# simplerr/rust-renderer

Hardware: AMD Instinct MI355X
Metric: Mrays/s (path rays: primary + bounce + sun-shadow + light-shadow) at 1920x1080, 20 spp = 20 frames x 1 spp; camera and sun at rest, the one-off builds of the camera grid and the sun grid outside the timed region (value_with_grid_builds charges them to these frames, value_tree_walk uses neither grid) (higher is better)
Workload: dtype f32

## Files before the change

rust-renderer_amd/csrc/context.hip:

```cpp
#include <hip/hip_runtime.h>
#include <rccl/rccl.h>
#include <dlfcn.h>

#include <algorithm>
#include <atomic>
#include <cstdlib>
#include <cmath>
#include <cstdio>
#include <cstring>
#include <string>
#include <vector>

#include "bvh.h"
#include "context_internal.h"
#include "context_state.h"
#include "device_scan.h"
#include "device_types.h"
#include "texture_layout.h"
#include "utopian_hip.h"

using namespace uh;

namespace {
std::string g_create_error;
// ... 344 lines not shown
   HIP_TRY(c, s.create(need));
   return UH_OK;
}

static int enqueue_path_trace(uh_ctx* c, Slot& s, const FrameParams& frame) {
   FrameParams fp = frame;
   LaunchCfg lc = cfg(c);
   lc.stream = s.stream;
   if (fp.batch_frames == 1) {
      lc.closest_blocks_per_cu = std::min(lc.closest_blocks_per_cu, uh_ctx::kSingleFrameBlocksPerCu);
      lc.shadow_blocks_per_cu = std::min(lc.shadow_blocks_per_cu, uh_ctx::kSingleFrameBlocksPerCu);
   }
   Control* ctl = s.control.p;
   DeviceStats* st = c->dstats.p;
   for (uint32_t smp = 0; smp < fp.samples_per_frame; smp++) {
      HIP_TRY(c, hipMemsetAsync(ctl, 0, sizeof(Control), s.stream));
      uint32_t slot = 0;
      launch_generate(lc, fp, s.ps, ctl, smp);
      const bool gpu_idle = !c->last_acc || hipEventQuery(c->last_acc) == hipSuccess;
      const bool fused = c->fused_bounces && fp.batch_frames == 1 && fp.num_bounces >= 2 && fp.num_bounces <= 64 && s.ps.shard_cap < (1u << 23) &&
                         ((gpu_idle && fp.n_owned <= uh_ctx::kFusedMaxPaths) || c->fused_always);
      const bool fused_sun0 = fused && fp.sun_shadow_enabled == 1 && fp.lights_enabled != 1;
      fp.sun_verdicts = (c->sun_x.verdicts && c->sun.this_frame && fp.sun_shadow_enabled == 1 && fp.lights_enabled != 1 && !fused) ? 1u : 0u;
      for (uint32_t b = 0; b < (fused ? 1u : fp.num_bounces); b++) {
         begin_timed(c, (b == 0 && c->cam.this_frame) ? 3 : 0, s.stream);
         if (b == 0 && c->cam.this_frame) {
            launch_trace_camera_grid(lc, fp, c->scene, s.ps, ctl, st, slot, slot + 1, c->cam.dev, c->cam.max_list_interior > std::max(c->cam.dev.walk_whole, c->cam.dev.max_walk));
            slot += 2;
         } else
            launch_trace_closest(lc, c->scene, s.ps, ctl, st, b, slot++, b == 0 ? UH_RAY_PRIMARY : UH_RAY_BOUNCE);
         end_timed(c, s.stream);
         const bool side_shadow = c->overlap_shadow && (fp.sun_shadow_enabled == 1 || fp.lights_enabled == 1);
         const bool side_used = side_shadow || c->overlap_miss;
         if (side_used && b > 0) HIP_TRY(c, hipStreamWaitEvent(s.stream, s.ev_shadowed, 0));
         begin_timed(c, 2, s.stream);
         launch_shade_hit(lc, fp, c->scene, s.ps, c->im, ctl, st, b);
         if (!c->overlap_miss) launch_shade_miss(lc, fp, s.ps, ctl, st, b);
         end_timed(c, s.stream);
// ... 32 lines not shown
      }
      const bool join_side = (c->overlap_miss || c->overlap_shadow) && fp.num_bounces > 0;
      if (join_side && !fused_sun0) {
         HIP_TRY(c, hipEventRecord(s.ev_side_done, s.side));
         HIP_TRY(c, hipStreamWaitEvent(s.stream, s.ev_side_done, 0));
      }
      if (fused) {
         begin_timed(c, 0, s.stream);
         launch_path_fused(lc, fp, c->scene, s.ps, ctl, st, c->sun.dev, c->sun.this_frame, fused_sun0);
         end_timed(c, s.stream);
      }
      if (join_side && fused_sun0) {
         HIP_TRY(c, hipEventRecord(s.ev_side_done, s.side));
         HIP_TRY(c, hipStreamWaitEvent(s.stream, s.ev_side_done, 0));
      }
      if (fp.num_bounces > 0 && !fused) launch_flush_survivors(lc, fp, s.ps, ctl);
      const bool last = smp + 1 == fp.samples_per_frame;
      if (last && c->last_acc && c->last_acc != s.ev_acc) HIP_TRY(c, hipStreamWaitEvent(s.stream, c->last_acc, 0));
      launch_finish_sample(lc, fp, s.ps, c->im, smp, last);
   }
   if (fp.samples_per_frame == 0) {
      if (c->last_acc && c->last_acc != s.ev_acc) HIP_TRY(c, hipStreamWaitEvent(s.stream, c->last_acc, 0));
      launch_resolve(lc, c->im, c->W, c->H, fp.total_samples, fp.accumulation_limit);
   }
   HIP_TRY(c, hipEventRecord(s.ev_acc, s.stream));
   c->last_acc = s.ev_acc;
   return UH_OK;
}

struct uh_batch {
   FrameParams fp;
// ... 498 lines not shown
   } else if (n == "sun_grid_max_mb") {
      if (!range(1, 65536)) return bad("must be 1..65536");
      c->sun.limits.max_entries = ((uint64_t)value << 20) / sizeof(SunGridEntry);
      c->sun.cache.invalidate();
   } else if (n == "sun_grid_force") {
      const SunGridLimits defaults;
      c->sun.limits.max_mean_list = value ? 1e30 : defaults.max_mean_list;
      c->sun.limits.max_fallback_area = value ? 2.0 : defaults.max_fallback_area;
      c->sun.cache.invalidate();
   } else if (n == "sun_grid_inline_max_mb") {
      if (!range(-1, 1 << 20)) return bad("must be -1 (auto: 4 x the packet array), 0 (off) .. 1048576");
      c->sun_x.inline_max_mb = value;
      c->sun.cache.invalidate();
   } else if (n == "sun_verdicts")
      c->sun_x.verdicts = value != 0;
   else if (n == "sun_grid_coarse") {
      if (!range(0, 6)) return bad("(log2 of the block edge in cells) must be 0..6");
      c->sun_x.coarse_shift = (uint32_t)value;
      c->sun.cache.invalidate();
   }
   else if (n == "camera_grid")
      c->cam_grid_enabled = value != 0;
   else if (n == "camera_grid_max_walk") {
      if (!range(1, 4096)) return bad("must be 1..4096");
      c->cam.limits.max_walk = (uint32_t)value;
      c->cam.cache.invalidate();
   } else if (n == "camera_grid_walk_whole") {
      if (!range(0, 65536)) return bad("must be 0..65536");
      c->cam_walk_whole = (uint32_t)value;
      c->cam.cache.invalidate();
// ... 385 lines not shown
```

rust-renderer_amd/csrc/context_state.h:

```cpp
#pragma once
#include <hip/hip_runtime.h>

#include <string>
#include <utility>
#include <vector>

#include "bvh.h"
#include "context_internal.h"
#include "device_types.h"
#include "grid_cache.h"
#include "utopian_hip.h"

using namespace uh;

struct HostMesh {
   std::vector<UhVertex> vertices;
   std::vector<uint32_t> indices;
   UhGpuMaterial material;
   float o2w[12];
   float w2o[9];
   bool iso = false, iso_reference = true;
   uint32_t iso_res = 0;
   float iso_lo = 0.0f, iso_hi = 0.0f;
   bool dev = false, host_valid = true;
// ... 108 lines not shown
   hipStream_t stream = nullptr;
   hipStream_t side = nullptr;
   hipEvent_t ev_traced = nullptr, ev_missed = nullptr, ev_shaded = nullptr, ev_shadowed = nullptr, ev_side_done = nullptr;
   hipEvent_t ev_acc = nullptr;
   hipEvent_t frame_start = nullptr, frame_stop = nullptr;
   DevBuf<float4> rec, radf, pixcol;
   DevBuf<uint32_t> queues[5];
   DevBuf<unsigned long long> sun_lit;
   DevBuf<Control> control;
   PathState ps{};
   bool ready = false;
   size_t capacity = 0;

   hipError_t create(size_t n) {
      capacity = n;
      uint32_t shard_cap = 0;
      {
         const uint32_t runs = (uint32_t)((n + 63) / 64);
         uint32_t per_shard[kShards] = {0};
         for (uint32_t r = 0; r < runs; r++) per_shard[shard_of_run(r)]++;
         for (uint32_t s = 0; s < kShards; s++) shard_cap = per_shard[s] * 64 > shard_cap ? per_shard[s] * 64 : shard_cap;
      }
      if (shard_cap >= (1u << 31)) return hipErrorInvalidValue;
      hipError_t e;
#define SLOT_TRY(expr)                 \
   if ((e = (expr)) != hipSuccess) return e
      SLOT_TRY(hipStreamCreateWithFlags(&stream, hipStreamNonBlocking));
      SLOT_TRY(hipStreamCreateWithFlags(&side, hipStreamNonBlocking));
      for (hipEvent_t* ev : {&ev_traced, &ev_missed, &ev_shaded, &ev_shadowed, &ev_side_done, &ev_acc}) SLOT_TRY(hipEventCreateWithFlags(ev, hipEventDisableTiming));
      SLOT_TRY(hipEventCreate(&frame_start));
      SLOT_TRY(hipEventCreate(&frame_stop));
      const size_t stagger = 4352;
      const size_t cap_q = (size_t)shard_cap * kShards;
      const size_t plane = (n > cap_q ? n : cap_q) + stagger / sizeof(float4);
      SLOT_TRY(rec.alloc(plane * (2 * kRecQuads + 1), 0 * stagger));
      SLOT_TRY(radf.alloc(n, 1 * stagger));
      SLOT_TRY(pixcol.alloc(n, 2 * stagger));
      for (int qi = 0; qi < 5; qi++) SLOT_TRY(queues[qi].alloc((size_t)shard_cap * kShards * (qi == 4 ? 2 : 1)));
      SLOT_TRY(sun_lit.alloc((size_t)shard_cap * kShards / 64));
      SLOT_TRY(hipMemsetAsync(sun_lit.p, 0, sun_lit.n * sizeof(unsigned long long), stream));
      SLOT_TRY(control.alloc(1));
      SLOT_TRY(hipMemsetAsync(control.p, 0, sizeof(Control), stream));
      SLOT_TRY(hipStreamSynchronize(stream));
#undef SLOT_TRY
      ps.set[0] = PathRecs{rec.p, plane};
      ps.set[1] = PathRecs{rec.p + plane * kRecQuads, plane};
      ps.hit = rec.p + plane * 2 * kRecQuads;
      ps.radf = radf.p;
      ps.pixcol = pixcol.p;
// ... 148 lines not shown
   uint32_t shadow_map_size = 4096;
   bool furnace = false;
   uint64_t frames = 0;
   float build_ms = 0.0f, last_frame_ms = 0.0f;
   float ms_by_kind[5] = {0, 0, 0, 0, 0};
   uint32_t trace_closest_launches = 0, trace_light_launches = 0;
   bool frame_timed = false;
   std::vector<EventPair> pending, free_events;
   uint32_t bvh_nodes = 0, bvh_tris = 0;

   bool sun_grid_enabled = true;
   uint64_t geom_version = 1;
   CachedGrid<3> sun;
   SunGridExtras sun_x;
   bool primary_implicit = true;

   bool cam_grid_enabled = true;
   CachedGrid<32> cam;

   uint32_t tp_rank = 0, tp_world = 1, tp_tile = 64;
   DevBuf<uint32_t> owned_pixels;
   uint32_t n_owned = 0;
   DevBuf<float4> tile_send, tile_recv;
   hipEvent_t ev_compose = nullptr;

   struct Hybrid {
      DevBuf<float4> pos, nrm, pbr;
      DevBuf<uchar4> alb, refl;
      DevBuf<uint8_t> shadow;
      DevBuf<uint32_t> queue, counter;
// ... 220 lines not shown
```

rust-renderer_amd/csrc/device_types.h:

```cpp
#pragma once
#include <hip/hip_runtime.h>

#include <cstdint>
#include <vector>

#include "bvh.h"
#include "post_levels.h"
#include "sun_grid.h"
#include "utopian_hip.h"

namespace uh {

constexpr uint32_t kMaxBounces = 64;
constexpr uint32_t kQueueKinds = 5;
enum { Q_RAY = 0, Q_LIGHT = 1, Q_SUN_TREE = 2, Q_MISS = 3, Q_CAM_TREE = 4 };
constexpr uint32_t kLaunchSlots = kMaxBounces * 4 + 8;

constexpr uint32_t kShards = 32;
constexpr uint32_t kShardBits = 5;
static_assert((1u << kShardBits) == kShards, "kShards is a power of two");
__host__ __device__ inline uint32_t shard_of_run(uint32_t run) { return (run * 0x9E3779B1u) >> (32 - kShardBits); }

constexpr uint32_t kBounceStride = ((kMaxBounces + 1 + 31) / 32) * 32;
constexpr uint32_t kSlotStride = ((kLaunchSlots + 31) / 32) * 32;
struct Control {
   uint32_t q_count[kShards * kQueueKinds * kBounceStride];
   uint32_t cursor[kShards * kSlotStride];
};
__host__ __device__ inline uint32_t qc_index(uint32_t bounce, uint32_t kind, uint32_t shard) { return (shard * kQueueKinds + kind) * kBounceStride + bounce; }
__host__ __device__ inline uint32_t cursor_index(uint32_t slot, uint32_t shard) { return shard * kSlotStride + slot; }

struct DeviceStats {
   unsigned long long rays[UH_RAY_KINDS];
   unsigned long long nodes_visited, tris_tested, shadow_nodes_visited, shadow_tris_tested;
   unsigned long long closest_hits, misses;
// ... 36 lines not shown

constexpr uint32_t kMaxBatchFrames = 32;

struct FrameParams {
   uint32_t batch_frames;
   uint32_t frame_numbers[kMaxBatchFrames];
   uint32_t total_samples_of[kMaxBatchFrames];
   const UhReservoir* spatial_of[kMaxBatchFrames];
   float inv_view[16], inv_proj[16], prev_pv[16];
   float sun_dir[3];
   uint32_t W, H, frame_number;
   uint32_t samples_per_frame, total_samples, num_bounces, accumulation_limit;
   uint32_t sky_enabled, sun_shadow_enabled, lights_enabled, use_ris, full_frame_restir;
   uint32_t primary_implicit;
   uint32_t sun_verdicts;
   uint32_t furnace;
   uint32_t num_lights_used;
   uint32_t temporal_enabled, spatial_enabled;
   uint32_t tp_rank, tp_world, tp_tile, tiles_x;
   const uint32_t* owned_pixels;
   uint32_t n_owned;
};

constexpr uint32_t kRecQuads = 4;
enum { REC_ORIGIN = 0, REC_DIR = 1, REC_THR = 2, REC_RAD = 3 };
struct PathRecs {
   float4* base;
   size_t plane;
};
struct PathState {
   PathRecs set[2];
   float4* hit;
   float4* radf;
   float4* pixcol;
   uint32_t* queue[5];
   unsigned long long* sun_lit;
   uint32_t shard_cap;
};
__host__ __device__ inline float4* rec_quad(const PathRecs& rec, uint32_t pos, int quad) { return rec.base + rec.plane * (size_t)quad + pos; }

struct RawRays {
   float4* ray_o;
   float4* ray_d;
   float4* hit;
};

struct Images {
   float4* accumulation;
   uchar4* output;
   float4* gbuffer_pos;
   UhReservoir* reservoirs[3];
   const UhReservoir* prev_spatial;
};

// ... 348 lines not shown
```

rust-renderer_amd/csrc/kernels.hip:

```cpp
#include <hip/hip_runtime.h>

#include "device_math.h"
#include "device_types.h"
#include "grid_walk.h"
#include "kernel_common.h"
#include "path_shading.h"
#include "traversal.h"

namespace uh {

template <bool COUNT>
__global__ __launch_bounds__(kBlock, 6) void k_trace_closest(SceneDev sc, bool sharded, const float4* __restrict__ ray_o,
                                                               const float4* __restrict__ ray_d, float4* __restrict__ hit_out, uint32_t shard_cap, Control* ctl,
                                                               DeviceStats* stats, uint32_t bounce, uint32_t cursor_slot, int ray_kind, uint32_t raw_count,
                                                               const uint32_t* __restrict__ listed) {
   const bool range_in_w = !sharded;
   __shared__ uint32_t s_stack[kWavesPerBlock][kLdsStack][64];
   __shared__ RayPool<2> s_pool[kWavesPerBlock];
   const uint32_t lane = lane_id();
   const uint32_t wave = threadIdx.x >> 6;
   uint32_t* lds_col = &s_stack[wave][0][lane];
   RayPool<2>& pool = s_pool[wave];
   RaySource src;
   uint32_t seg = 0;
// ... 30 lines not shown
      trav_init(t, ro, rd, range_in_w ? ro.w : 0.001f, range_in_w ? rd.w : 10000.0f, INFINITY);
   };
   while (refill_lanes<2>(f, src, pool, t.cur == kEmptyRef, source_of, take)) {
      if (t.cur != kEmptyRef) {
         bool occluded = false;
         if (trav_step<false, COUNT>(nodes, tris, t, lds_col, spill, occluded, n_nodes, n_tris))
            st_rec(hit_out + where, make_float4(t.best.t, t.best.u, t.best.v, __uint_as_float(t.best.idx)));
      }
   }
   if (COUNT) {
      atomicAdd(&stats->nodes_visited, (unsigned long long)n_nodes);
      atomicAdd(&stats->tris_tested, (unsigned long long)n_tris);
   }
}

template <bool COUNT, bool LIGHT, bool VERDICT = false>
__global__ __launch_bounds__(kBlock, 5) void k_trace_shadow(SceneDev sc, FrameParams fp, PathState ps, Control* ctl, DeviceStats* stats, uint32_t bounce,
                                                              uint32_t cursor_slot, bool leftovers) {
   __shared__ uint32_t s_stack[kWavesPerBlock][kLdsStack][64];
   static_assert(!(VERDICT && LIGHT), "verdicts are the sun rays'");
   constexpr int NA = VERDICT ? 1 : 3;
   __shared__ RayPool<NA> s_pool[kWavesPerBlock];
   const uint32_t lane = lane_id();
   const uint32_t wave = threadIdx.x >> 6;
   uint32_t* lds_col = &s_stack[wave][0][lane];
   RayPool<NA>& pool = s_pool[wave];
   const ShardCtx sx = shard_ctx();
   const uint32_t seg = sx.shard * ps.shard_cap;
   RaySource src;
   src.queue = LIGHT ? ps.queue[2] + seg : leftovers ? ps.queue[3] + seg : nullptr;
   src.count = LIGHT ? ctl->q_count[qc_index(bounce, Q_LIGHT, sx.shard)] : leftovers ? ctl->q_count[qc_index(bounce, Q_SUN_TREE, sx.shard)] : ctl->q_count[qc_index(bounce + 1, Q_RAY, sx.shard)];
   src.cursor = &ctl->cursor[cursor_index(cursor_slot, sx.shard)];
   src.wave_index = src.num_waves = 0;
   if (sx.lb == 0 && threadIdx.x == 0) {
      if (!leftovers) atomicAdd(&stats->rays[LIGHT ? UH_RAY_LIGHT_SHADOW : UH_RAY_SUN_SHADOW], (unsigned long long)src.count);
      else if (src.count) atomicAdd(&stats->sun_tree_rays, (unsigned long long)src.count);
   }
   const uint4* __restrict__ nodes = sc.nodes;
   const float4* __restrict__ tris = sc.tris;
   const PathRecs rec = ps.set[(bounce + 1) & 1];
   float4* rad = rec_quad(rec, seg, REC_RAD);
   auto source_of = [&](int a, uint32_t pos) { return (const float4*)rec_quad(rec, seg + pos, a == 0 ? REC_ORIGIN : a == 1 ? REC_THR : REC_RAD); };
   Feeder<NA> f;
   Trav t;
   t.cur = kEmptyRef;
   t.sp = 0;
   uint32_t id = 0, n_nodes = 0, n_tris = 0;
   float4 lit = make_float4(0.0f, 0.0f, 0.0f, 0.0f);
   uint32_t spill[kSpillStack];
   auto take = [&](uint32_t slot) {
      id = pool.id[slot];
      ShadowRay s;
      if constexpr (VERDICT) {
         s = make_shadow_ray<false>(sc, fp, pool.v[0][slot], 0u);
      } else {
         const float4 thr = pool.v[1][slot], r4 = pool.v[2][slot];
         s = make_shadow_ray<LIGHT>(sc, fp, pool.v[0][slot], __float_as_uint(r4.w));
         lit = shadow_lit<LIGHT>(thr, r4);
      }
      trav_init(t, s.ro, s.rd, s.ro.w, s.rd.w, s.tlimit);
   };
   while (refill_lanes<NA>(f, src, pool, t.cur == kEmptyRef, source_of, take)) {
      if (t.cur != kEmptyRef) {
         bool occluded = false;
         if (trav_step<true, COUNT>(nodes, tris, t, lds_col, spill, occluded, n_nodes, n_tris) && !occluded) {
            if constexpr (VERDICT)
               atomicOr(sun_lit_word(ps, seg + id), 1ull << (id & 63u));
            else
               st_stream(rad + id, lit);
         }
      }
   }
   if (COUNT) {
      atomicAdd(LIGHT ? &stats->light_nodes_visited : &stats->shadow_nodes_visited, (unsigned long long)n_nodes);
      atomicAdd(LIGHT ? &stats->light_tris_tested : &stats->shadow_tris_tested, (unsigned long long)n_tris);
   }
}

template <bool COUNT, bool INLINE, bool VERDICT>
__global__ __launch_bounds__(kBlock) void k_trace_sun_grid(SceneDev sc, FrameParams fp, PathState ps, Control* ctl, DeviceStats* stats, uint32_t bounce,
                                                            uint32_t cursor_slot, SunGridDev g) {
   const uint32_t lane = lane_id();
   const ShardCtx sx = shard_ctx();
   const uint32_t seg = sx.shard * ps.shard_cap;
   const PathRecs rec = ps.set[(bounce + 1) & 1];
   const uint32_t count = ctl->q_count[qc_index(bounce + 1, Q_RAY, sx.shard)];
   uint32_t* cursor = &ctl->cursor[cursor_index(cursor_slot, sx.shard)];
   const V3 d = v3(fp.sun_dir[0], fp.sun_dir[1], fp.sun_dir[2]);
   uint32_t n_tris = 0, n_covered = 0;
   uint32_t* q_tree = ps.queue[3] + seg;
   uint32_t* n_tree = &ctl->q_count[qc_index(bounce, Q_SUN_TREE, sx.shard)];
   constexpr int K = kSunRaysPerLane;
   typedef float f4_t __attribute__((ext_vector_type(4)));
   const f4_t* __restrict__ recs = reinterpret_cast<const f4_t*>(g.recs);
// ... 124 lines not shown
                  }
                  e++;
                  if (e >= end[k] || __uint_as_float(nx.y) < pw[k]) break;
                  cur = nx;
                  if (e + 1 < end[k]) nx = entries[e + 1];
                  const f4_t* r = tris + kTriStride16 * (size_t)cur.x;
                  const f4_t na = r[0], nb = r[1], nc = r[2];
                  a = make_float4(na.x, na.y, na.z, na.w);
                  b = make_float4(nb.x, nb.y, nb.z, nb.w);
                  c = make_float4(nc.x, nc.y, nc.z, nc.w);
               }
            }
            lit[k] = !occluded;
         }
      });
      if constexpr (VERDICT) {
         static_for<K>([&](auto kc) {
            constexpr int k = decltype(kc)::value;
            const unsigned long long word = __ballot(lit[k]);
            if (lane == 0 && base + 64u * k < count) *sun_lit_word(ps, seg + base + 64u * k) = word;
         });
      } else {
         float4 thr[K], rad[K];
         static_for<K>([&](auto kc) {
            constexpr int k = decltype(kc)::value;
            if (lit[k]) {
               thr[k] = ld_rec(rec_quad(rec, seg + id[k], REC_THR));
               rad[k] = ld_rec(rec_quad(rec, seg + id[k], REC_RAD));
            }
         });
         static_for<K>([&](auto kc) {
// ... 140 lines not shown
   for (uint32_t g = blockIdx.x * kWavesPerBlock + (threadIdx.x >> 6); g < groups; g += gridDim.x * kWavesPerBlock) {
      const uint32_t q = g * 64u + lane;
      bool own = q < n;
      uint32_t id = 0;
      float4 s_o = make_float4(0, 0, 0, 0), s_d = make_float4(0, 0, 0, 0);
      if (own) id = q;
      if (own && !fp.primary_implicit) {
         const uint32_t f = q / fp.n_owned, k = q - f * fp.n_owned;
         const uint32_t pix = fp.owned_pixels ? fp.owned_pixels[k] : k;
         uint32_t px = pix % fp.W, py = pix / fp.W;
         uint32_t rng = sample == 0 ? init_rng(px, py, fp.W, fp.frame_numbers[f]) : __float_as_uint(ps.radf[id].w);
         uint32_t seed = rng;
         float jx = random_float(rng), jy = random_float(rng);
         V3 o, d;
         primary_ray(fp, px, py, jx, jy, o, d);
         s_o = make_float4(o.x, o.y, o.z, __uint_as_float(rng));
         s_d = make_float4(d.x, d.y, d.z, __uint_as_float(seed));
      }
      uint32_t shard = own ? shard_of_run(id >> 6) : 0xffffffffu;
      unsigned long long todo = __ballot(own);
      while (todo) {
         const int leader = __ffsll((long long)todo) - 1;
         const uint32_t s = __shfl(shard, leader);
         const bool mine = own && shard == s;
         uint32_t slot = wave_append(&ctl->q_count[qc_index(0, Q_RAY, s)], mine);
         if (mine) {
            const uint32_t pos = s * ps.shard_cap + slot;
            ps.queue[0][pos] = id;
            if (!fp.primary_implicit) {
               st_rec(rec_quad(ps.set[0], pos, REC_ORIGIN), s_o);
               st_rec(rec_quad(ps.set[0], pos, REC_DIR), s_d);
               st_rec(rec_quad(ps.set[0], pos, REC_THR), make_float4(1.0f, 1.0f, 1.0f, 0.0f));
            }
         }
         todo &= ~__ballot(mine);
      }
   }
}

__global__ __launch_bounds__(kBlock) void k_shade_miss(FrameParams fp, PathState ps, Control* ctl, DeviceStats* stats, uint32_t bounce) {
   const ShardCtx sx = shard_ctx();
   const uint32_t seg = sx.shard * ps.shard_cap;
   const uint2* __restrict__ queue = reinterpret_cast<const uint2*>(ps.queue[4]) + seg;
   const uint32_t count = ctl->q_count[qc_index(bounce, Q_MISS, sx.shard)];
   for (uint32_t i = sx.lb * kBlock + threadIdx.x; i < count; i += sx.nb * kBlock) {
      const uint2 e = ld_stream(queue + i);
      shade_miss_path(fp, ps, seg + (e.x & ~kSunLitBit), e.y, bounce, (e.x & kSunLitBit) != 0u);
   }
   if (sx.lb == 0 && threadIdx.x == 0 && count) atomicAdd(&stats->misses, (unsigned long long)count);
}

__global__ __launch_bounds__(kBlock, kShadeHitBlocks) void k_shade_hit(FrameParams fp, SceneDev sc, PathState ps, Control* ctl, DeviceStats* stats, uint32_t bounce) {
   __shared__ float s_lut[256];
   s_lut[threadIdx.x] = sc.unorm_lut[threadIdx.x];
   constexpr uint32_t kLdsMeshes = 192, kLdsTextures = 64;
   __shared__ MeshShade s_mesh[kLdsMeshes];
   __shared__ TexInfo s_tex[kLdsTextures];
   const uint32_t n_lds_mesh = sc.num_meshes < kLdsMeshes ? sc.num_meshes : kLdsMeshes;
   const uint32_t n_lds_tex = sc.num_textures < kLdsTextures ? sc.num_textures : kLdsTextures;
   __shared__ uint32_t s_hits;
   __shared__ uint32_t s_list[kWavesPerBlock][6][128];
   __shared__ uint32_t s_miss[kWavesPerBlock][2][128];
   if (threadIdx.x == 0) s_hits = 0;
   if (threadIdx.x < n_lds_mesh) s_mesh[threadIdx.x] = sc.meshes[threadIdx.x];
   if (threadIdx.x < n_lds_tex) s_tex[threadIdx.x] = sc.textures[threadIdx.x];
   __syncthreads();
// ... 17 lines not shown
      const uint32_t pk = __float_as_uint(hr.w);
      bool scattered = false, want_light = false;
      uint32_t slot = 0;
      float4 n_o = make_float4(0, 0, 0, 0), n_d = make_float4(0, 0, 0, 0), n_t = make_float4(0, 0, 0, 0), n_r = make_float4(0, 0, 0, 0);
      if (valid) {
         float4 ro, rd, thr4;
         if (bounce == 0 && fp.primary_implicit) {
            primary_state(fp, id, ro, rd);
            thr4 = make_float4(1.0f, 1.0f, 1.0f, 0.0f);
         } else {
            ro = ld_rec(rec_quad(cur, seg + pos, REC_ORIGIN));
            rd = ld_rec(rec_quad(cur, seg + pos, REC_DIR));
            thr4 = ld_rec(rec_quad(cur, seg + pos, REC_THR));
         }
         uint2 rng = make_uint2(__float_as_uint(ro.w), __float_as_uint(rd.w));
         float4 rad4 = make_float4(0.0f, 0.0f, 0.0f, 0.0f);
         if (rad_stored(fp, bounce)) rad4 = ld_rec(rec_quad(cur, seg + pos, REC_RAD));
         const V3 ray_dir = v3(rd.x, rd.y, rd.z);
         const float t = hr.x, bu = hr.y, bv = hr.z;
         const float4* sp = sc.shade + 4 * (size_t)pk;
         float4 s0 = sp[0], s1 = sp[1], s2 = sp[2], s3 = sp[3];
         const uint32_t mesh_index = __float_as_uint(s3.w);
         MeshShade ms = lds_fetch(s_mesh + (mesh_index < kLdsMeshes ? mesh_index : kLdsMeshes - 1));
         if (mesh_index >= n_lds_mesh) ms = sc.meshes[mesh_index];
         V3 normal;
         float uu, vv;
         surface_normal_uv(s0, s1, s2, s3, bu, bv, normal, uu, vv);
         asm volatile("" : "+v"(rng.x), "+v"(rng.y), "+v"(thr4.x), "+v"(thr4.y), "+v"(thr4.z), "+v"(rad4.x), "+v"(rad4.y), "+v"(rad4.z));
         if (sun_lit) rad4 = shadow_lit<false>(thr4, rad4);
         const V3 world_normal = world_normal_of(ms, normal, ray_dir);
         V3 origin = v3(ro.x, ro.y, ro.z) + t * ray_dir;
         origin = offset_ray(origin, world_normal);
// ... 8 lines not shown
            if (scattered && (int)lane_id() == scat_leader) scat_base = __hip_atomic_fetch_add(counter, (uint32_t)__popcll(scat_mask), __ATOMIC_RELAXED, __HIP_MEMORY_SCOPE_AGENT);
         });
         color = color * v3(ms.base_color[0], ms.base_color[1], ms.base_color[2]);

         uint32_t seed = rng.y;
         const V3 scatter = material_scatter(ms, ray_dir, world_normal, color, seed);
         rng.y = seed;
         if (scat_leader >= 0) slot = (uint32_t)__builtin_amdgcn_readlane((int)scat_base, scat_leader) + __builtin_amdgcn_mbcnt_hi((uint32_t)(scat_mask >> 32), __builtin_amdgcn_mbcnt_lo((uint32_t)scat_mask, 0u));

         V3 thr = v3(thr4.x, thr4.y, thr4.z) * color;
         if (!scattered) {
            st_stream(ps.radf + id, make_float4(rad4.x + thr.x, rad4.y + thr.y, rad4.z + thr.z, __uint_as_float(rng.x)));
         } else {
            float f = 0.0f;
            int light_index = 0;
            if (fp.lights_enabled == 1) want_light = select_light(fp, sc, id, rng.x, origin, f, light_index);
            n_o = make_float4(origin.x, origin.y, origin.z, __uint_as_float(rng.x));
            n_d = make_float4(scatter.x, scatter.y, scatter.z, __uint_as_float(rng.y));
            n_t = make_float4(thr.x, thr.y, thr.z, f);
            n_r = make_float4(rad4.x, rad4.y, rad4.z, __uint_as_float((uint32_t)light_index));
         }
      }
      const uint32_t lslot = wave_append(n_light, want_light);
      if (scattered) {
         st_stream(q_next + slot, id);
         st_rec(rec_quad(nxt, seg + slot, REC_ORIGIN), n_o);
         if (bounce + 1 < fp.num_bounces) st_rec(rec_quad(nxt, seg + slot, REC_DIR), n_d);
         st_rec(rec_quad(nxt, seg + slot, REC_THR), n_t);
         if (rad_stored(fp, bounce + 1)) st_rec(rec_quad(nxt, seg + slot, REC_RAD), n_r);
      }
      if (want_light) st_stream(q_light + lslot, slot);
   };
   uint32_t(*list)[128] = s_list[threadIdx.x >> 6];
   uint32_t(*missed)[128] = s_miss[threadIdx.x >> 6];
   const uint32_t lane = lane_id();
   uint32_t n_list = 0, n_missed = 0;
   const bool verdicts = bounce != 0 && fp.sun_verdicts != 0;
   auto flush_misses = [&](uint32_t n) {
      uint32_t base = 0;
      if (lane == 0) base = atomicAdd(n_miss, n);
      base = __shfl(base, 0);
      if (lane < n) st_stream(q_miss + base + lane, make_uint2(missed[0][lane], missed[1][lane]));
   };
   auto entry = [&](uint32_t k) { return make_float4(__uint_as_float(list[2][k]), __uint_as_float(list[3][k]), __uint_as_float(list[4][k]), __uint_as_float(list[5][k])); };
   for (uint32_t r = 0; r < rounds; r++) {
      const uint32_t i = r * stride + sx.lb * kBlock + threadIdx.x;
      uint32_t id = 0;
      float4 hr = make_float4(0.0f, 0.0f, 0.0f, __uint_as_float(kEmptyRef));
      if (i < count) {
         id = ld_stream(queue + i);
         hr = ld_rec(ps.hit + seg + i);
      }
      uint32_t i_lit = i;
      if (verdicts) {
         const uint32_t i0 = __builtin_amdgcn_readfirstlane(i - lane);
         if (i0 < count && ((*sun_lit_word(ps, seg + i0) >> lane) & 1ull)) i_lit |= kSunLitBit;
      }
      const bool is_hit = __float_as_uint(hr.w) != kEmptyRef;
      const unsigned long long mask = __ballot(is_hit);
      const unsigned long long mmask = __ballot(i < count && !is_hit);
      if (mmask) {
         const uint32_t mp = __builtin_amdgcn_mbcnt_hi((uint32_t)(mmask >> 32), __builtin_amdgcn_mbcnt_lo((uint32_t)mmask, 0u));
         if (i < count && !is_hit) {
            missed[0][n_missed + mp] = i_lit;
            missed[1][n_missed + mp] = id;
// ... 8 lines not shown
               tmp0 = missed[0][64u + lane];
               tmp1 = missed[1][64u + lane];
            }
            __builtin_amdgcn_wave_barrier();
            if (lane < rest) {
               missed[0][lane] = tmp0;
               missed[1][lane] = tmp1;
            }
            __builtin_amdgcn_wave_barrier();
            n_missed = rest;
         }
      }
      if (mask == 0ull) continue;
      const uint32_t prefix = __builtin_amdgcn_mbcnt_hi((uint32_t)(mask >> 32), __builtin_amdgcn_mbcnt_lo((uint32_t)mask, 0u));
      if (is_hit) {
         list[0][n_list + prefix] = id;
         list[1][n_list + prefix] = i_lit;
         list[2][n_list + prefix] = __float_as_uint(hr.x);
         list[3][n_list + prefix] = __float_as_uint(hr.y);
         list[4][n_list + prefix] = __float_as_uint(hr.z);
         list[5][n_list + prefix] = __float_as_uint(hr.w);
      }
      n_list += (uint32_t)__popcll(mask);
      __builtin_amdgcn_wave_barrier();
      if (n_list >= 64u) {
         shade(list[0][lane], list[1][lane], entry(lane), true);
         n_hits += 64u;
         const uint32_t rest = n_list - 64u;
         uint32_t tmp[6] = {0, 0, 0, 0, 0, 0};
         if (lane < rest)
            for (int k = 0; k < 6; k++) tmp[k] = list[k][64u + lane];
// ... 127 lines not shown

void launch_trace_camera_grid(const LaunchCfg& c, const FrameParams& fp, const SceneDev& sc, const PathState& ps, Control* ctl, DeviceStats* stats, uint32_t cursor_slot_grid,
                              uint32_t cursor_slot_tree, const SunGridDev& g, bool leftovers_possible) {
   const dim3 grid = sharded_grid(c.num_cus * 8);
   if (c.count_visits)
      k_trace_camera_grid<true><<<grid, kBlock, 0, c.stream>>>(sc, fp, ps, ctl, stats, cursor_slot_grid, g);
   else
      k_trace_camera_grid<false><<<grid, kBlock, 0, c.stream>>>(sc, fp, ps, ctl, stats, cursor_slot_grid, g);
   if (!leftovers_possible) return;
   const PathRecs& rec = ps.set[0];
   launch_closest(c, closest_grid(c), sc, true, rec_quad(rec, 0, REC_ORIGIN), rec_quad(rec, 0, REC_DIR), ps.hit, ps.shard_cap, ctl, stats, 0, cursor_slot_tree, UH_RAY_PRIMARY, 0, ps.queue[3]);
}

void launch_shade_miss(const LaunchCfg& c, const FrameParams& fp, const PathState& ps, Control* ctl, DeviceStats* stats, uint32_t bounce) {
   const dim3 full = shade_grid(c, fp.n_owned * fp.batch_frames), lean = sharded_grid(c.num_cus * 8);
   k_shade_miss<<<full.x < lean.x ? full : lean, kBlock, 0, c.stream>>>(fp, ps, ctl, stats, bounce);
}

void launch_shade_hit(const LaunchCfg& c, const FrameParams& fp, const SceneDev& sc, const PathState& ps, const Images& im, Control* ctl,
                      DeviceStats* stats, uint32_t bounce) {
   k_shade_hit<<<shade_grid(c, fp.W * fp.H), kBlock, 0, c.stream>>>(fp, sc, ps, ctl, stats, bounce);
}
void launch_flush_survivors(const LaunchCfg& c, const FrameParams& fp, const PathState& ps, Control* ctl) {
   k_flush_survivors<<<shade_grid(c, fp.n_owned * fp.batch_frames), kBlock, 0, c.stream>>>(fp, ps, ctl);
}

void launch_trace_shadow(const LaunchCfg& c, const FrameParams& fp, const SceneDev& sc, const PathState& ps, Control* ctl, DeviceStats* stats,
                         uint32_t bounce, uint32_t cursor_slot, bool light, bool sun_leftovers) {
   as_constant(c.count_visits, [&](auto count) {
      auto go = [&](auto is_light, auto verdict) {
         k_trace_shadow<decltype(count)::value, decltype(is_light)::value, decltype(verdict)::value><<<shadow_grid(c), kBlock, 0, c.stream>>>(
            sc, fp, ps, ctl, stats, bounce, cursor_slot, sun_leftovers);
      };
      if (light) go(std::true_type{}, std::false_type{});
      else if (sun_leftovers && fp.sun_verdicts) go(std::false_type{}, std::true_type{});
      else go(std::false_type{}, std::false_type{});
   });
}

void launch_trace_sun_grid(const LaunchCfg& c, const FrameParams& fp, const SceneDev& sc, const PathState& ps, Control* ctl, DeviceStats* stats, uint32_t bounce,
                           uint32_t cursor_slot, const SunGridDev& g) {
   const dim3 grid = sharded_grid(c.num_cus * 8);
   as_constant(c.count_visits, [&](auto count) {
      as_constant(g.recs != nullptr, [&](auto inl) {
         as_constant(fp.sun_verdicts != 0, [&](auto verdict) {
            k_trace_sun_grid<decltype(count)::value, decltype(inl)::value, decltype(verdict)::value><<<grid, kBlock, 0, c.stream>>>(
               sc, fp, ps, ctl, stats, bounce, cursor_slot, g);
         });
      });
   });
}

void launch_finish_sample(const LaunchCfg& c, const FrameParams& fp, const PathState& ps, const Images& im, uint32_t sample, bool last) {
   k_finish_sample<<<stream_grid(c, fp.n_owned), kBlock, 0, c.stream>>>(fp, ps, im, sample, last);
}

void launch_resolve(const LaunchCfg& c, const Images& im, uint32_t W, uint32_t H, uint32_t total_samples, uint32_t limit) {
   k_resolve<<<stream_grid(c, W * H), kBlock, 0, c.stream>>>(im, W * H, total_samples, limit);
}

void launch_gbuffer_cast(const LaunchCfg& c, const FrameParams& fp, const SceneDev& sc, const RawRays& rr, const RowSpans& spans, DeviceStats* stats,
                         const SunGridDev* camera_grid) {
   const uint32_t n = spans.total();
// ... 27 lines not shown
```

rust-renderer_amd/csrc/path_shading.h:

```cpp
#pragma once
#include <hip/hip_runtime.h>

#include "device_math.h"
#include "device_types.h"

namespace uh {

struct ShadowRay {
   float4 ro, rd;
   float tlimit;
};
template <bool LIGHT>
__device__ __forceinline__ ShadowRay make_shadow_ray(const SceneDev& sc, const FrameParams& fp, float4 ro, uint32_t light_bits) {
   ShadowRay s;
   s.ro = make_float4(ro.x, ro.y, ro.z, 0.001f);
   s.tlimit = INFINITY;
   if (LIGHT) {
      const int light_index = (int)light_bits;
      V3 lpos = v3(0, 0, 0);
      if (light_index >= 0 && (uint32_t)light_index < sc.num_lights) lpos = xyz(sc.lights[2 * light_index]);
      const V3 o = v3(ro.x, ro.y, ro.z);
      const V3 dir = normalize3(lpos - o);
      s.tlimit = length3(lpos - o);
      s.rd = make_float4(dir.x, dir.y, dir.z, 10000.0f);
// ... 1 lines not shown
      s.rd = make_float4(fp.sun_dir[0], fp.sun_dir[1], fp.sun_dir[2], 10000.0f);
   }
   return s;
}
template <bool LIGHT>
__device__ __forceinline__ float4 shadow_lit(float4 thr, float4 rad) {
   if (LIGHT) {
      const float f = thr.w;
      return make_float4(rad.x + thr.x * f, rad.y + thr.y * f, rad.z + thr.z * f, rad.w);
   }
   return make_float4(rad.x + thr.x, rad.y + thr.y, rad.z + thr.z, rad.w);
}
__device__ __forceinline__ unsigned long long* sun_lit_word(const PathState& ps, uint32_t pos) { return ps.sun_lit + (pos >> 6); }
__device__ __forceinline__ bool rad_stored(const FrameParams& fp, uint32_t b) { return b > fp.sun_verdicts; }
constexpr uint32_t kSunLitBit = 0x80000000u;

__device__ __forceinline__ void shade_miss_path(const FrameParams& fp, const PathState& ps, uint32_t pos, uint32_t id, uint32_t bounce, bool sun_lit) {
   const PathRecs rec = ps.set[bounce & 1];
   const bool implicit = bounce == 0 && fp.primary_implicit;
   float4 ro, rd_implicit = make_float4(0.0f, 0.0f, 0.0f, 0.0f);
   if (implicit)
      primary_state(fp, id, ro, rd_implicit);
   else
      ro = ld_rec(rec_quad(rec, pos, REC_ORIGIN));
   V3 sky_color = v3(0.0f, 0.0f, 0.0f);
   if (fp.furnace) {
      sky_color = v3(1.0f, 1.0f, 1.0f);
   } else if (fp.sky_enabled == 1) {
      const float4 rd = implicit ? rd_implicit : ld_rec(rec_quad(rec, pos, REC_DIR));
      V3 c = sky::integrate_scattering(v3(ro.x, ro.y, ro.z), v3(rd.x, rd.y, rd.z), 999999999.0f, v3(fp.sun_dir[0], fp.sun_dir[1], fp.sun_dir[2]));
      sky_color = v3(fminf(c.x, 1.0f), fminf(c.y, 1.0f), fminf(c.z, 1.0f));
   }
   float4 thr = make_float4(1.0f, 1.0f, 1.0f, 0.0f);
   if (!implicit) thr = ld_rec(rec_quad(rec, pos, REC_THR));
   float4 rad = make_float4(0.0f, 0.0f, 0.0f, 0.0f);
   if (rad_stored(fp, bounce)) rad = ld_rec(rec_quad(rec, pos, REC_RAD));
   if (sun_lit) rad = shadow_lit<false>(thr, rad);
   V3 t = v3(thr.x, thr.y, thr.z) * sky_color;
   st_stream(ps.radf + id, make_float4(rad.x + t.x, rad.y + t.y, rad.z + t.z, ro.w));
}

__device__ __forceinline__ V3 pbr_weight(V3 N, V3 V, V3 L, V3 base, float metallic, float roughness) {
   const float PI = 3.14159265359f;
   const V3 H = normalize3(V + L);
   const float a = roughness * roughness, a2 = a * a;
   const float NdotH = fmaxf(dot3(N, H), 0.0f), NdotH2 = NdotH * NdotH;
   float denom = NdotH2 * (a2 - 1.0f) + 1.0f;
   denom = (PI * denom) * denom;
   const float NDF = a2 / denom;
   const float NdotV = fmaxf(dot3(N, V), 0.0f), NdotL = fmaxf(dot3(N, L), 0.0f);
   const float r = roughness + 1.0f, k = (r * r) / 8.0f;
// ... 108 lines not shown
```

Measured before the change: 10430.

## Add slim path state: pack radiance, carry path id in origin, write final radiance

Adds a default-on slim_state mode for sun-verdict single-sample frames. Path id travels in the origin's w slot instead of a separate queue, and the radiance record shrinks to a float2 (green, blue) with red kept in throughput's w. The last bounce's sun-shadow kernels write the final radiance straight to radf, so the flush-survivors pass is skipped. The aim is less per-bounce memory traffic and one fewer kernel. In exchange, light sampling (RIS) is disabled on this path and the RNG state in origin.w is dropped (rng.x is zeroed), which could affect correctness.

```diff
diff --git a/rust-renderer_amd/csrc/context.hip b/rust-renderer_amd/csrc/context.hip
--- a/rust-renderer_amd/csrc/context.hip
+++ b/rust-renderer_amd/csrc/context.hip
@@ -382,14 +382,15 @@
    Control* ctl = s.control.p;
    DeviceStats* st = c->dstats.p;
    for (uint32_t smp = 0; smp < fp.samples_per_frame; smp++) {
-      HIP_TRY(c, hipMemsetAsync(ctl, 0, sizeof(Control), s.stream));
       uint32_t slot = 0;
-      launch_generate(lc, fp, s.ps, ctl, smp);
       const bool gpu_idle = !c->last_acc || hipEventQuery(c->last_acc) == hipSuccess;
       const bool fused = c->fused_bounces && fp.batch_frames == 1 && fp.num_bounces >= 2 && fp.num_bounces <= 64 && s.ps.shard_cap < (1u << 23) &&
                          ((gpu_idle && fp.n_owned <= uh_ctx::kFusedMaxPaths) || c->fused_always);
       const bool fused_sun0 = fused && fp.sun_shadow_enabled == 1 && fp.lights_enabled != 1;
       fp.sun_verdicts = (c->sun_x.verdicts && c->sun.this_frame && fp.sun_shadow_enabled == 1 && fp.lights_enabled != 1 && !fused) ? 1u : 0u;
+      fp.slim_state = (c->slim_state && fp.sun_verdicts == 1 && fp.samples_per_frame == 1) ? 1u : 0u;
+      HIP_TRY(c, hipMemsetAsync(ctl, 0, sizeof(Control), s.stream));
+      launch_generate(lc, fp, s.ps, ctl, smp);
       for (uint32_t b = 0; b < (fused ? 1u : fp.num_bounces); b++) {
          begin_timed(c, (b == 0 && c->cam.this_frame) ? 3 : 0, s.stream);
          if (b == 0 && c->cam.this_frame) {
@@ -452,7 +453,7 @@
          HIP_TRY(c, hipEventRecord(s.ev_side_done, s.side));
          HIP_TRY(c, hipStreamWaitEvent(s.stream, s.ev_side_done, 0));
       }
-      if (fp.num_bounces > 0 && !fused) launch_flush_survivors(lc, fp, s.ps, ctl);
+      if (fp.num_bounces > 0 && !fused && !fp.slim_state) launch_flush_survivors(lc, fp, s.ps, ctl);
       const bool last = smp + 1 == fp.samples_per_frame;
       if (last && c->last_acc && c->last_acc != s.ev_acc) HIP_TRY(c, hipStreamWaitEvent(s.stream, c->last_acc, 0));
       launch_finish_sample(lc, fp, s.ps, c->im, smp, last);
@@ -981,6 +982,8 @@
       c->sun.cache.invalidate();
    } else if (n == "sun_verdicts")
       c->sun_x.verdicts = value != 0;
+   else if (n == "slim_state")
+      c->slim_state = value != 0;
    else if (n == "sun_grid_coarse") {
       if (!range(0, 6)) return bad("(log2 of the block edge in cells) must be 0..6");
       c->sun_x.coarse_shift = (uint32_t)value;
diff --git a/rust-renderer_amd/csrc/context_state.h b/rust-renderer_amd/csrc/context_state.h
--- a/rust-renderer_amd/csrc/context_state.h
+++ b/rust-renderer_amd/csrc/context_state.h
@@ -146,13 +146,7 @@
 
    hipError_t create(size_t n) {
       capacity = n;
-      uint32_t shard_cap = 0;
-      {
-         const uint32_t runs = (uint32_t)((n + 63) / 64);
-         uint32_t per_shard[kShards] = {0};
-         for (uint32_t r = 0; r < runs; r++) per_shard[shard_of_run(r)]++;
-         for (uint32_t s = 0; s < kShards; s++) shard_cap = per_shard[s] * 64 > shard_cap ? per_shard[s] * 64 : shard_cap;
-      }
+      const uint32_t shard_cap = layout_shard_cap(n);
       if (shard_cap >= (1u << 31)) return hipErrorInvalidValue;
       hipError_t e;
 #define SLOT_TRY(expr)                 \
@@ -162,9 +156,8 @@
       for (hipEvent_t* ev : {&ev_traced, &ev_missed, &ev_shaded, &ev_shadowed, &ev_side_done, &ev_acc}) SLOT_TRY(hipEventCreateWithFlags(ev, hipEventDisableTiming));
       SLOT_TRY(hipEventCreate(&frame_start));
       SLOT_TRY(hipEventCreate(&frame_stop));
-      const size_t stagger = 4352;
-      const size_t cap_q = (size_t)shard_cap * kShards;
-      const size_t plane = (n > cap_q ? n : cap_q) + stagger / sizeof(float4);
+      const size_t stagger = kPlaneStaggerBytes;
+      const size_t plane = layout_plane_quads(n, shard_cap);
       SLOT_TRY(rec.alloc(plane * (2 * kRecQuads + 1), 0 * stagger));
       SLOT_TRY(radf.alloc(n, 1 * stagger));
       SLOT_TRY(pixcol.alloc(n, 2 * stagger));
@@ -343,6 +336,7 @@
    CachedGrid<3> sun;
    SunGridExtras sun_x;
    bool primary_implicit = true;
+   bool slim_state = true;
 
    bool cam_grid_enabled = true;
    CachedGrid<32> cam;
diff --git a/rust-renderer_amd/csrc/device_types.h b/rust-renderer_amd/csrc/device_types.h
--- a/rust-renderer_amd/csrc/device_types.h
+++ b/rust-renderer_amd/csrc/device_types.h
@@ -5,6 +5,7 @@
 #include <vector>
 
 #include "bvh.h"
+#include "path_layout.h"
 #include "post_levels.h"
 #include "sun_grid.h"
 #include "utopian_hip.h"
@@ -19,6 +20,7 @@
 constexpr uint32_t kShards = 32;
 constexpr uint32_t kShardBits = 5;
 static_assert((1u << kShardBits) == kShards, "kShards is a power of two");
+static_assert(kLayoutShards == kShards && kLayoutShardBits == kShardBits, "path_layout.h states the same shards");
 __host__ __device__ inline uint32_t shard_of_run(uint32_t run) { return (run * 0x9E3779B1u) >> (32 - kShardBits); }
 
 constexpr uint32_t kBounceStride = ((kMaxBounces + 1 + 31) / 32) * 32;
@@ -85,6 +87,7 @@
    uint32_t sky_enabled, sun_shadow_enabled, lights_enabled, use_ris, full_frame_restir;
    uint32_t primary_implicit;
    uint32_t sun_verdicts;
+   uint32_t slim_state;
    uint32_t furnace;
    uint32_t num_lights_used;
    uint32_t temporal_enabled, spatial_enabled;
@@ -108,7 +111,12 @@
    unsigned long long* sun_lit;
    uint32_t shard_cap;
 };
-__host__ __device__ inline float4* rec_quad(const PathRecs& rec, uint32_t pos, int quad) { return rec.base + rec.plane * (size_t)quad + pos; }
+__host__ __device__ inline float4* rec_quad(const PathRecs& rec, uint32_t pos, int quad) {
+   return reinterpret_cast<float4*>(reinterpret_cast<char*>(rec.base) + rec_offset(rec.plane, pos, quad));
+}
+__host__ __device__ inline float2* rec_pair(const PathRecs& rec, uint32_t pos) {
+   return reinterpret_cast<float2*>(reinterpret_cast<char*>(rec.base) + rec_offset(rec.plane, pos, REC_RAD, true));
+}
 
 struct RawRays {
    float4* ray_o;
diff --git a/rust-renderer_amd/csrc/kernels.hip b/rust-renderer_amd/csrc/kernels.hip
--- a/rust-renderer_amd/csrc/kernels.hip
+++ b/rust-renderer_amd/csrc/kernels.hip
@@ -68,11 +68,12 @@
    }
 }
 
-template <bool COUNT, bool LIGHT, bool VERDICT = false>
+template <bool COUNT, bool LIGHT, bool VERDICT = false, bool FINAL = false>
 __global__ __launch_bounds__(kBlock, 5) void k_trace_shadow(SceneDev sc, FrameParams fp, PathState ps, Control* ctl, DeviceStats* stats, uint32_t bounce,
                                                               uint32_t cursor_slot, bool leftovers) {
    __shared__ uint32_t s_stack[kWavesPerBlock][kLdsStack][64];
    static_assert(!(VERDICT && LIGHT), "verdicts are the sun rays'");
+   static_assert(VERDICT || !FINAL, "the final form replaces the verdict");
    constexpr int NA = VERDICT ? 1 : 3;
    __shared__ RayPool<NA> s_pool[kWavesPerBlock];
    const uint32_t lane = lane_id();
@@ -100,6 +101,7 @@
    t.cur = kEmptyRef;
    t.sp = 0;
    uint32_t id = 0, n_nodes = 0, n_tris = 0;
+   uint32_t path_id = 0;
    float4 lit = make_float4(0.0f, 0.0f, 0.0f, 0.0f);
    uint32_t spill[kSpillStack];
    auto take = [&](uint32_t slot) {
@@ -107,6 +109,7 @@
       ShadowRay s;
       if constexpr (VERDICT) {
          s = make_shadow_ray<false>(sc, fp, pool.v[0][slot], 0u);
+         if constexpr (FINAL) path_id = __float_as_uint(pool.v[0][slot].w);
       } else {
          const float4 thr = pool.v[1][slot], r4 = pool.v[2][slot];
          s = make_shadow_ray<LIGHT>(sc, fp, pool.v[0][slot], __float_as_uint(r4.w));
@@ -117,7 +120,16 @@
    while (refill_lanes<NA>(f, src, pool, t.cur == kEmptyRef, source_of, take)) {
       if (t.cur != kEmptyRef) {
          bool occluded = false;
-         if (trav_step<true, COUNT>(nodes, tris, t, lds_col, spill, occluded, n_nodes, n_tris) && !occluded) {
+         const bool ended = trav_step<true, COUNT>(nodes, tris, t, lds_col, spill, occluded, n_nodes, n_tris);
+         if constexpr (FINAL) {
+            if (ended) {
+               const float4 thr = ld_rec(rec_quad(rec, seg + id, REC_THR));
+               float4 r = make_float4(0.0f, 0.0f, 0.0f, 0.0f);
+               if (rad_stored(fp, bounce + 1)) r = ld_rad<true>(rec, seg + id, thr);
+               if (!occluded) r = shadow_lit<false>(thr, r);
+               st_stream(ps.radf + path_id, make_float4(r.x, r.y, r.z, 0.0f));
+            }
+         } else if (ended && !occluded) {
             if constexpr (VERDICT)
                atomicOr(sun_lit_word(ps, seg + id), 1ull << (id & 63u));
             else
@@ -131,7 +143,7 @@
    }
 }
 
-template <bool COUNT, bool INLINE, bool VERDICT>
+template <bool COUNT, bool INLINE, bool VERDICT, bool FINAL = false>
 __global__ __launch_bounds__(kBlock) void k_trace_sun_grid(SceneDev sc, FrameParams fp, PathState ps, Control* ctl, DeviceStats* stats, uint32_t bounce,
                                                             uint32_t cursor_slot, SunGridDev g) {
    const uint32_t lane = lane_id();
@@ -286,7 +298,26 @@
             lit[k] = !occluded;
          }
       });
-      if constexpr (VERDICT) {
+      if constexpr (FINAL) {
+         static_assert(VERDICT, "the final form replaces the verdict");
+         const bool stored = rad_stored(fp, bounce + 1);
+         float4 thr[K], rad[K];
+         static_for<K>([&](auto kc) {
+            constexpr int k = decltype(kc)::value;
+            rad[k] = make_float4(0.0f, 0.0f, 0.0f, 0.0f);
+            if (valid[k] && !defer[k]) {
+               thr[k] = ld_rec(rec_quad(rec, seg + id[k], REC_THR));
+               if (stored) rad[k] = ld_rad<true>(rec, seg + id[k], thr[k]);
+            }
+         });
+         static_for<K>([&](auto kc) {
+            constexpr int k = decltype(kc)::value;
+            if (valid[k] && !defer[k]) {
+               if (lit[k]) rad[k] = shadow_lit<false>(thr[k], rad[k]);
+               st_stream(ps.radf + __float_as_uint(ro[k].w), make_float4(rad[k].x, rad[k].y, rad[k].z, 0.0f));
+            }
+         });
+      } else if constexpr (VERDICT) {
          static_for<K>([&](auto kc) {
             constexpr int k = decltype(kc)::value;
             const unsigned long long word = __ballot(lit[k]);
@@ -457,7 +488,7 @@
          float jx = random_float(rng), jy = random_float(rng);
          V3 o, d;
          primary_ray(fp, px, py, jx, jy, o, d);
-         s_o = make_float4(o.x, o.y, o.z, __uint_as_float(rng));
+         s_o = make_float4(o.x, o.y, o.z, __uint_as_float(fp.slim_state ? id : rng));
          s_d = make_float4(d.x, d.y, d.z, __uint_as_float(seed));
       }
       uint32_t shard = own ? shard_of_run(id >> 6) : 0xffffffffu;
@@ -481,6 +512,7 @@
    }
 }
 
+template <bool SLIM>
 __global__ __launch_bounds__(kBlock) void k_shade_miss(FrameParams fp, PathState ps, Control* ctl, DeviceStats* stats, uint32_t bounce) {
    const ShardCtx sx = shard_ctx();
    const uint32_t seg = sx.shard * ps.shard_cap;
@@ -488,11 +520,12 @@
    const uint32_t count = ctl->q_count[qc_index(bounce, Q_MISS, sx.shard)];
    for (uint32_t i = sx.lb * kBlock + threadIdx.x; i < count; i += sx.nb * kBlock) {
       const uint2 e = ld_stream(queue + i);
-      shade_miss_path(fp, ps, seg + (e.x & ~kSunLitBit), e.y, bounce, (e.x & kSunLitBit) != 0u);
+      shade_miss_path<SLIM>(fp, ps, seg + (e.x & ~kSunLitBit), e.y, bounce, (e.x & kSunLitBit) != 0u);
    }
    if (sx.lb == 0 && threadIdx.x == 0 && count) atomicAdd(&stats->misses, (unsigned long long)count);
 }
 
+template <bool SLIM>
 __global__ __launch_bounds__(kBlock, kShadeHitBlocks) void k_shade_hit(FrameParams fp, SceneDev sc, PathState ps, Control* ctl, DeviceStats* stats, uint32_t bounce) {
    __shared__ float s_lut[256];
    s_lut[threadIdx.x] = sc.unorm_lut[threadIdx.x];
@@ -540,8 +573,12 @@
             thr4 = ld_rec(rec_quad(cur, seg + pos, REC_THR));
          }
          uint2 rng = make_uint2(__float_as_uint(ro.w), __float_as_uint(rd.w));
+         if constexpr (SLIM) {
+            if (bounce != 0) id = rng.x;
+            rng.x = 0u;
+         }
          float4 rad4 = make_float4(0.0f, 0.0f, 0.0f, 0.0f);
-         if (rad_stored(fp, bounce)) rad4 = ld_rec(rec_quad(cur, seg + pos, REC_RAD));
+         if (rad_stored(fp, bounce)) rad4 = ld_rad<SLIM>(cur, seg + pos, thr4);
          const V3 ray_dir = v3(rd.x, rd.y, rd.z);
          const float t = hr.x, bu = hr.y, bv = hr.z;
          const float4* sp = sc.shade + 4 * (size_t)pk;
@@ -580,20 +617,25 @@
          } else {
             float f = 0.0f;
             int light_index = 0;
-            if (fp.lights_enabled == 1) want_light = select_light(fp, sc, id, rng.x, origin, f, light_index);
-            n_o = make_float4(origin.x, origin.y, origin.z, __uint_as_float(rng.x));
+            if constexpr (!SLIM)
+               if (fp.lights_enabled == 1) want_light = select_light(fp, sc, id, rng.x, origin, f, light_index);
+            n_o = make_float4(origin.x, origin.y, origin.z, __uint_as_float(SLIM ? id : rng.x));
             n_d = make_float4(scatter.x, scatter.y, scatter.z, __uint_as_float(rng.y));
-            n_t = make_float4(thr.x, thr.y, thr.z, f);
+            n_t = make_float4(thr.x, thr.y, thr.z, SLIM ? rad4.x : f);
             n_r = make_float4(rad4.x, rad4.y, rad4.z, __uint_as_float((uint32_t)light_index));
          }
       }
-      const uint32_t lslot = wave_append(n_light, want_light);
+      uint32_t lslot = 0;
+      if constexpr (!SLIM) lslot = wave_append(n_light, want_light);
       if (scattered) {
-         st_stream(q_next + slot, id);
+         if constexpr (!SLIM) st_stream(q_next + slot, id);
          st_rec(rec_quad(nxt, seg + slot, REC_ORIGIN), n_o);
          if (bounce + 1 < fp.num_bounces) st_rec(rec_quad(nxt, seg + slot, REC_DIR), n_d);
          st_rec(rec_quad(nxt, seg + slot, REC_THR), n_t);
-         if (rad_stored(fp, bounce + 1)) st_rec(rec_quad(nxt, seg + slot, REC_RAD), n_r);
+         if (rad_stored(fp, bounce + 1)) {
+            if constexpr (SLIM) st_rad_pair(nxt, seg + slot, n_r.y, n_r.z);
+            else st_rec(rec_quad(nxt, seg + slot, REC_RAD), n_r);
+         }
       }
       if (want_light) st_stream(q_light + lslot, slot);
    };
@@ -614,7 +656,7 @@
       uint32_t id = 0;
       float4 hr = make_float4(0.0f, 0.0f, 0.0f, __uint_as_float(kEmptyRef));
       if (i < count) {
-         id = ld_stream(queue + i);
+         if (!SLIM || bounce == 0) id = ld_stream(queue + i);
          hr = ld_rec(ps.hit + seg + i);
       }
       uint32_t i_lit = i;
@@ -653,7 +695,7 @@
       if (mask == 0ull) continue;
       const uint32_t prefix = __builtin_amdgcn_mbcnt_hi((uint32_t)(mask >> 32), __builtin_amdgcn_mbcnt_lo((uint32_t)mask, 0u));
       if (is_hit) {
-         list[0][n_list + prefix] = id;
+         if (!SLIM || bounce == 0) list[0][n_list + prefix] = id;
          list[1][n_list + prefix] = i_lit;
          list[2][n_list + prefix] = __float_as_uint(hr.x);
          list[3][n_list + prefix] = __float_as_uint(hr.y);
@@ -811,13 +853,15 @@
 
 void launch_shade_miss(const LaunchCfg& c, const FrameParams& fp, const PathState& ps, Control* ctl, DeviceStats* stats, uint32_t bounce) {
    const dim3 full = shade_grid(c, fp.n_owned * fp.batch_frames), lean = sharded_grid(c.num_cus * 8);
-   k_shade_miss<<<full.x < lean.x ? full : lean, kBlock, 0, c.stream>>>(fp, ps, ctl, stats, bounce);
+   as_constant(fp.slim_state != 0, [&](auto slim) { k_shade_miss<decltype(slim)::value><<<full.x < lean.x ? full : lean, kBlock, 0, c.stream>>>(fp, ps, ctl, stats, bounce); });
 }
 
 void launch_shade_hit(const LaunchCfg& c, const FrameParams& fp, const SceneDev& sc, const PathState& ps, const Images& im, Control* ctl,
                       DeviceStats* stats, uint32_t bounce) {
-   k_shade_hit<<<shade_grid(c, fp.W * fp.H), kBlock, 0, c.stream>>>(fp, sc, ps, ctl, stats, bounce);
-}
+   as_constant(fp.slim_state != 0, [&](auto slim) { k_shade_hit<decltype(slim)::value><<<shade_grid(c, fp.W * fp.H), kBlock, 0, c.stream>>>(fp, sc, ps, ctl, stats, bounce); });
+}
+static bool final_sun_rays(const FrameParams& fp, uint32_t bounce) { return fp.slim_state != 0 && bounce + 1 == fp.num_bounces; }
+
 void launch_flush_survivors(const LaunchCfg& c, const FrameParams& fp, const PathState& ps, Control* ctl) {
    k_flush_survivors<<<shade_grid(c, fp.n_owned * fp.batch_frames), kBlock, 0, c.stream>>>(fp, ps, ctl);
 }
@@ -825,13 +869,14 @@
 void launch_trace_shadow(const LaunchCfg& c, const FrameParams& fp, const SceneDev& sc, const PathState& ps, Control* ctl, DeviceStats* stats,
                          uint32_t bounce, uint32_t cursor_slot, bool light, bool sun_leftovers) {
    as_constant(c.count_visits, [&](auto count) {
-      auto go = [&](auto is_light, auto verdict) {
-         k_trace_shadow<decltype(count)::value, decltype(is_light)::value, decltype(verdict)::value><<<shadow_grid(c), kBlock, 0, c.stream>>>(
+      auto go = [&](auto is_light, auto verdict, auto final) {
+         k_trace_shadow<decltype(count)::value, decltype(is_light)::value, decltype(verdict)::value, decltype(final)::value><<<shadow_grid(c), kBlock, 0, c.stream>>>(
             sc, fp, ps, ctl, stats, bounce, cursor_slot, sun_leftovers);
       };
-      if (light) go(std::true_type{}, std::false_type{});
-      else if (sun_leftovers && fp.sun_verdicts) go(std::false_type{}, std::true_type{});
-      else go(std::false_type{}, std::false_type{});
+      if (light) go(std::true_type{}, std::false_type{}, std::false_type{});
+      else if (sun_leftovers && final_sun_rays(fp, bounce)) go(std::false_type{}, std::true_type{}, std::true_type{});
+      else if (sun_leftovers && fp.sun_verdicts) go(std::false_type{}, std::true_type{}, std::false_type{});
+      else go(std::false_type{}, std::false_type{}, std::false_type{});
    });
 }
 
@@ -840,10 +885,13 @@
    const dim3 grid = sharded_grid(c.num_cus * 8);
    as_constant(c.count_visits, [&](auto count) {
       as_constant(g.recs != nullptr, [&](auto inl) {
-         as_constant(fp.sun_verdicts != 0, [&](auto verdict) {
-            k_trace_sun_grid<decltype(count)::value, decltype(inl)::value, decltype(verdict)::value><<<grid, kBlock, 0, c.stream>>>(
+         auto go = [&](auto verdict, auto final) {
+            k_trace_sun_grid<decltype(count)::value, decltype(inl)::value, decltype(verdict)::value, decltype(final)::value><<<grid, kBlock, 0, c.stream>>>(
                sc, fp, ps, ctl, stats, bounce, cursor_slot, g);
-         });
+         };
+         if (final_sun_rays(fp, bounce)) go(std::true_type{}, std::true_type{});
+         else if (fp.sun_verdicts != 0) go(std::true_type{}, std::false_type{});
+         else go(std::false_type{}, std::false_type{});
       });
    });
 }
diff --git a/rust-renderer_amd/csrc/path_layout.h b/rust-renderer_amd/csrc/path_layout.h
--- /dev/null
+++ b/rust-renderer_amd/csrc/path_layout.h
@@ -0,0 +1,36 @@
+#pragma once
+#include <cstddef>
+#include <cstdint>
+
+#if defined(__HIPCC__)
+#define UH_LAYOUT_HD __host__ __device__
+#else
+#define UH_LAYOUT_HD
+#endif
+
+namespace uh {
+
+constexpr uint32_t kLayoutShards = 32;
+constexpr uint32_t kLayoutShardBits = 5;
+constexpr uint32_t kRecQuadBytes = 16, kRecPairBytes = 8;
+constexpr size_t kPlaneStaggerBytes = 4352;
+
+UH_LAYOUT_HD inline uint32_t layout_shard_of_run(uint32_t run) { return (run * 0x9E3779B1u) >> (32 - kLayoutShardBits); }
+
+inline uint32_t layout_shard_cap(size_t n) {
+   const uint32_t runs = (uint32_t)((n + 63) / 64);
+   uint32_t per_shard[kLayoutShards] = {0}, cap = 0;
+   for (uint32_t r = 0; r < runs; r++) per_shard[layout_shard_of_run(r)]++;
+   for (uint32_t s = 0; s < kLayoutShards; s++) cap = per_shard[s] * 64 > cap ? per_shard[s] * 64 : cap;
+   return cap;
+}
+inline size_t layout_plane_quads(size_t n, uint32_t shard_cap) {
+   const size_t cap_q = (size_t)shard_cap * kLayoutShards;
+   return (n > cap_q ? n : cap_q) + kPlaneStaggerBytes / kRecQuadBytes;
+}
+
+UH_LAYOUT_HD inline size_t rec_offset(size_t plane, uint32_t pos, int quad, bool pairs = false) {
+   return (plane * (size_t)quad) * kRecQuadBytes + (size_t)pos * ((pairs && quad == 3) ? kRecPairBytes : kRecQuadBytes);
+}
+
+}
diff --git a/rust-renderer_amd/csrc/path_shading.h b/rust-renderer_amd/csrc/path_shading.h
--- a/rust-renderer_amd/csrc/path_shading.h
+++ b/rust-renderer_amd/csrc/path_shading.h
@@ -39,7 +39,21 @@
 __device__ __forceinline__ unsigned long long* sun_lit_word(const PathState& ps, uint32_t pos) { return ps.sun_lit + (pos >> 6); }
 __device__ __forceinline__ bool rad_stored(const FrameParams& fp, uint32_t b) { return b > fp.sun_verdicts; }
 constexpr uint32_t kSunLitBit = 0x80000000u;
-
+typedef float v2f_t __attribute__((ext_vector_type(2)));
+template <bool SLIM>
+__device__ __forceinline__ float4 ld_rad(const PathRecs& rec, uint32_t pos, float4 thr) {
+   if constexpr (SLIM) {
+      const v2f_t gb = __builtin_nontemporal_load(reinterpret_cast<const v2f_t*>(rec_pair(rec, pos)));
+      return make_float4(thr.w, gb.x, gb.y, 0.0f);
+   } else
+      return ld_rec(rec_quad(rec, pos, REC_RAD));
+}
+__device__ __forceinline__ void st_rad_pair(const PathRecs& rec, uint32_t pos, float g, float b) {
+   const v2f_t gb = {g, b};
+   __builtin_nontemporal_store(gb, reinterpret_cast<v2f_t*>(rec_pair(rec, pos)));
+}
+
+template <bool SLIM = false>
 __device__ __forceinline__ void shade_miss_path(const FrameParams& fp, const PathState& ps, uint32_t pos, uint32_t id, uint32_t bounce, bool sun_lit) {
    const PathRecs rec = ps.set[bounce & 1];
    const bool implicit = bounce == 0 && fp.primary_implicit;
@@ -48,6 +62,10 @@
       primary_state(fp, id, ro, rd_implicit);
    else
       ro = ld_rec(rec_quad(rec, pos, REC_ORIGIN));
+   if constexpr (SLIM) {
+      if (bounce != 0) id = __float_as_uint(ro.w);
+      ro.w = 0.0f;
+   }
    V3 sky_color = v3(0.0f, 0.0f, 0.0f);
    if (fp.furnace) {
       sky_color = v3(1.0f, 1.0f, 1.0f);
@@ -59,7 +77,7 @@
    float4 thr = make_float4(1.0f, 1.0f, 1.0f, 0.0f);
    if (!implicit) thr = ld_rec(rec_quad(rec, pos, REC_THR));
    float4 rad = make_float4(0.0f, 0.0f, 0.0f, 0.0f);
-   if (rad_stored(fp, bounce)) rad = ld_rec(rec_quad(rec, pos, REC_RAD));
+   if (rad_stored(fp, bounce)) rad = ld_rad<SLIM>(rec, pos, thr);
    if (sun_lit) rad = shadow_lit<false>(thr, rad);
    V3 t = v3(thr.x, thr.y, thr.z) * sky_color;
    st_stream(ps.radf + id, make_float4(rad.x + t.x, rad.y + t.y, rad.z + t.z, ro.w));
```

After: 10680, median of 6. 1.02x the previous value.
